# johanngerberding/voxelnet-pytorch

Hardware: AMD Instinct MI355X
Metric: point-clouds/sec fwd+bwd, KITTI car voxel grid, batch=2 (higher is better)
Workload: dtype bf16; 1 GPU; KITTI car config (voxel 0.2x0.2x0.4 m, grid 10x400x352, T=35), batch=2 per GPU, fwd+bwd train step (BASELINE configs[1]); global_batch=2, points_per_frame=19861, parallelism=dp1, launch_mode=eager+native-executor+one-call-step

## Files before the change

### voxelnet-pytorch_amd/csrc/conv.hip

```cpp
#include "common.h"

namespace {

constexpr int GG_MAX_TAPS = 32;
constexpr int GG_MAX_CLASSES = 16;
constexpr uint32_t GG_OOB = 0xFFFFF000u;
constexpr uint32_t GG_MAX_WINDOW = 0xFFFFE000u;

struct GGClass {
    int32_t tap_begin, ntaps;
    int32_t nD, nH, nW;
    int32_t qD, qH, qW;
    int32_t ooffD, ooffH, ooffW;
    int32_t offD[4], offH[4], offW[4];
};
struct GGTap {
    int32_t id, ih, iw, widx;
};
struct GGParams {
    const char *src;
    const char *w;
    const float *bias;
    char *out;
    float *stats;
// ... 10 lines not shown
    uint32_t w_bytes;
    int64_t src_batch_extent;
    const int64_t *row_list;
    const int32_t *row_count;
    int32_t row_cap;
    int32_t out_linear;
    int32_t ldivD, ldivH, ldivW;
    int32_t slotcD[4], slotcH[4], slotcW[4];
    GGClass cls[GG_MAX_CLASSES];
    GGTap taps[GG_MAX_TAPS];
};

typedef __attribute__((address_space(3))) void lds_void_t;
#ifdef VN_P2D_TRACE
__device__ long long g_p2d_trace[64 * 8];
#define P2D_STAMP(s, k) do { if (tr_on) g_p2d_trace[((s) & 63) * 8 + (k)] = __builtin_amdgcn_s_memtime(); } while (0)
#else
#define P2D_STAMP(s, k) do {} while (0)
#endif
#ifndef GG_PIN_SCHEDULE
#define GG_PIN_SCHEDULE 1
#endif
#if GG_PIN_SCHEDULE
#define GG_PIN() __builtin_amdgcn_sched_barrier(0)
#else
#define GG_PIN()
#endif

__device__ __forceinline__ void lds_dma16(__amdgpu_buffer_rsrc_t rsrc, char *lds_wave_base, uint32_t voffset,
                                          uint32_t soffset) {
    __builtin_amdgcn_raw_ptr_buffer_load_lds(rsrc, (lds_void_t *)lds_wave_base, 16, voffset, soffset, 0, 0);
}

__device__ __forceinline__ void x3_weights(bool presplit, const char *g0, const char *g1, bf16x8_t &hi, bf16x8_t &lo) {
    if (presplit) {
        hi = *reinterpret_cast<const bf16x8_t *>(g0);
        lo = *reinterpret_cast<const bf16x8_t *>(g1);
    } else {
        vn_split8(*reinterpret_cast<const f32x4_t *>(g0), *reinterpret_cast<const f32x4_t *>(g1), hi, lo);
    }
}

template <int NT>
__device__ __forceinline__ void x3_split_patch(char *patch, int rows) {
    for (int item = threadIdx.x; item < rows * 4; item += NT) {
        const int q = item >> 2, f = item & 3, sw = (q >> 1) & 7;
        char *g0 = patch + q * 128 + (((2 * f) ^ sw) << 4), *g1 = patch + q * 128 + (((2 * f + 1) ^ sw) << 4);
        bf16x8_t hi, lo;
        vn_split8(*reinterpret_cast<const f32x4_t *>(g0), *reinterpret_cast<const f32x4_t *>(g1), hi, lo);
        *reinterpret_cast<bf16x8_t *>(g0) = hi;
        *reinterpret_cast<bf16x8_t *>(g1) = lo;
    }
}

template <int WM, int WN, int SM, bool BNBWD = false>
__device__ __forceinline__ void gg_store(const GGParams &p, f32x4_t (&acc)[SM][4], char *smem, const int32_t *otab, int64_t tile,
                                         int n0, int wm, int wn, int lane) {
    constexpr int BN = 64 * WN;
    const int fr = lane & 15, fq = lane >> 4;
    const int64_t tile_m = tile;
    const int ncol = n0 + wn * 64 + fr * 4;
    const bool col_ok = ncol < p.N;
    float bias4[4] = {0.f, 0.f, 0.f, 0.f};
    if (p.bias && col_ok) {
        const float4 bv = *reinterpret_cast<const float4 *>(p.bias + ncol);
        bias4[0] = bv.x; bias4[1] = bv.y; bias4[2] = bv.z; bias4[3] = bv.w;
    }
    float s1[4] = {0.f, 0.f, 0.f, 0.f}, s2[4] = {0.f, 0.f, 0.f, 0.f};
    float bmean[4] = {0.f, 0.f, 0.f, 0.f}, binv[4] = {0.f, 0.f, 0.f, 0.f}, bS[4] = {0.f, 0.f, 0.f, 0.f}, bbe[4] = {0.f, 0.f, 0.f, 0.f};
    if constexpr (BNBWD) {
        if (col_ok) {
#pragma unroll
            for (int j = 0; j < 4; ++j) {
                bmean[j] = p.bn_stats[ncol + j]; binv[j] = p.bn_stats[p.N + ncol + j];
                bS[j] = p.bn_stats[2 * p.N + ncol + j]; bbe[j] = p.bn_stats[3 * p.N + ncol + j];
            }
        }
    }
#pragma unroll
    for (int i = 0; i < SM; ++i) {
        const int4 offs = *reinterpret_cast<const int4 *>(otab + wm * (16 * SM) + i * 16 + fq * 4);
        const int32_t o4[4] = {offs.x, offs.y, offs.z, offs.w};
#pragma unroll
        for (int e = 0; e < 4; ++e) {
            if (o4[e] < 0 || !col_ok) continue;
            float v[4];
            if constexpr (BNBWD) {
                float yv[4];
                if (p.bn_y_f32) {
                    const float4 t = *reinterpret_cast<const float4 *>(reinterpret_cast<const float *>(p.bn_y) + (int64_t)o4[e] + ncol);
                    yv[0] = t.x; yv[1] = t.y; yv[2] = t.z; yv[3] = t.w;
                } else {
                    const bf16x4_t t = *reinterpret_cast<const bf16x4_t *>(reinterpret_cast<const bf16_t *>(p.bn_y) + (int64_t)o4[e] + ncol);
#pragma unroll
                    for (int j = 0; j < 4; ++j) yv[j] = (float)t[j];
                }
#pragma unroll
                for (int j = 0; j < 4; ++j) {
                    const float a = acc[i][j][e];
                    v[j] = a;
                    const float st = p.out_f32 ? a : (float)(bf16_t)a;
                    const float d0 = yv[j] - bmean[j];
                    const float z = fmaf(bS[j], d0, bbe[j]);
                    const float dz = z > 0.f ? st : 0.f;
                    s1[j] += dz;
                    s2[j] += dz * (d0 * binv[j]);
                }
            } else {
#pragma unroll
            for (int j = 0; j < 4; ++j) {
                const float a = acc[i][j][e];
                s1[j] += a;
                s2[j] += a * a;
                v[j] = a + bias4[j];
            }
            }
            if (p.out_f32) {
                float4 *dst = reinterpret_cast<float4 *>(reinterpret_cast<float *>(p.out) + (int64_t)o4[e] + ncol);
                if (p.accumulate) {
                    const float4 old = *dst;
                    v[0] += old.x; v[1] += old.y; v[2] += old.z; v[3] += old.w;
                }
                *dst = make_float4(v[0], v[1], v[2], v[3]);
            } else {
                bf16x4_t *dst = reinterpret_cast<bf16x4_t *>(reinterpret_cast<bf16_t *>(p.out) + (int64_t)o4[e] + ncol);
                if (p.accumulate) {
                    const bf16x4_t old = *dst;
#pragma unroll
                    for (int j = 0; j < 4; ++j) v[j] += (float)old[j];
                }
                bf16x4_t o;
#pragma unroll
                for (int j = 0; j < 4; ++j) o[j] = (bf16_t)v[j];
                *dst = o;
            }
        }
    }
    if (p.stats) {
        __syncthreads();
        float *red = reinterpret_cast<float *>(smem);
#pragma unroll
        for (int j = 0; j < 4; ++j) {
            s1[j] += __shfl_xor(s1[j], 16, 64);
            s1[j] += __shfl_xor(s1[j], 32, 64);
            s2[j] += __shfl_xor(s2[j], 16, 64);
            s2[j] += __shfl_xor(s2[j], 32, 64);
        }
        if (fq == 0) {
#pragma unroll
            for (int j = 0; j < 4; ++j) {
                red[(wm * 2 + 0) * BN + wn * 64 + fr * 4 + j] = s1[j];
                red[(wm * 2 + 1) * BN + wn * 64 + fr * 4 + j] = s2[j];
            }
        }
        __syncthreads();
        for (int i = threadIdx.x; i < 2 * BN; i += 64 * WM * WN) {
            const int which = i / BN, c = i - which * BN;
            float v = 0.f;
#pragma unroll
            for (int w = 0; w < WM; ++w) v += red[(w * 2 + which) * BN + c];
            if (n0 + c < p.N) p.stats[((int64_t)tile_m * 2 + which) * p.N + n0 + c] = v;
        }
    }
}

template <int WM, int WN, int SM, int NS, bool F32>
__global__ void __launch_bounds__(256, 2) k_gather_gemm(const GGParams p) {
    VN_PRIO_MAIN();
    static_assert(WM * WN == 4 && NS >= 2 && SM >= 1 && SM <= 8, "4 waves");
    constexpr int ESZ = F32 ? 4 : 2;
    constexpr int BM = 16 * SM * WM, BN = 64 * WN;
    static_assert(BM % 32 == 0, "a DMA instruction of the 4 waves covers 32 rows");
    constexpr int RA = BM / 32, RB = BN / 32;
    constexpr int A_BYTES = BM * 128, B_BYTES = BN * 128, STAGE = A_BYTES + B_BYTES;
    constexpr int AHEAD = (NS - 2) * (RA + RB);
    static_assert(AHEAD <= 63, "vmcnt is 6 bits");
    extern __shared__ __attribute__((aligned(16))) char smem[];

    const int lane = threadIdx.x & 63;
    const int wave = __builtin_amdgcn_readfirstlane(threadIdx.x >> 6);
    const int wm = wave / WN, wn = wave % WN;

    const GGClass &cl = p.cls[blockIdx.y];
    const int ntn = (p.N + BN - 1) / BN;
    int bid = blockIdx.x;
    {
        const int nwg = gridDim.x, q = nwg >> 3, r = nwg & 7, x = bid & 7;
        bid = (x < r ? x * (q + 1) : r * (q + 1) + (x - r) * q) + (bid >> 3);
    }
    const int tile_m = bid / ntn, tile_n = bid - tile_m * ntn;
    const int qD = cl.qD, qH = cl.qH, qW = cl.qW;
    const bool list = p.row_list != nullptr;
    const int64_t Mq = list ? (p.row_count ? (int64_t)p.row_count[0] : (int64_t)p.row_cap) : (int64_t)p.B * qD * qH * qW;
    const int64_t m0 = (int64_t)tile_m * BM;
    const int n0 = tile_n * BN;
    if (m0 >= Mq) {
// ... 227 lines not shown
        nbuf = nbuf + 1 == NS ? 0 : nbuf + 1;
    }

    __syncthreads();
    int32_t *otab = reinterpret_cast<int32_t *>(smem);
    for (int r = threadIdx.x; r < BM; r += 256) {
        const int64_t m = m0 + r;
        int32_t off = -1;
        if (m < Mq && list) {
            if (p.out_linear) {
                off = (int32_t)(m * p.oW);
            } else {
                const int64_t *rc = p.row_list + m * 4;
                off = (int32_t)(rc[0] * p.oB + rc[1] * p.oD + rc[2] * p.oH + rc[3] * p.oW);
            }
        } else if (m < Mq) {
            int t = (int)(m % rows_per_b);
            const int b = (int)(m / rows_per_b);
            const int qw = t % qW;
            t /= qW;
            const int qh = t % qH;
            const int qd = t / qH;
            const int od = qd * p.omulD + cl.ooffD, oh = qh * p.omulH + cl.ooffH, ow = qw * p.omulW + cl.ooffW;
            if (od < p.Do && oh < p.Ho && ow < p.Wo)
                off = (int32_t)((int64_t)b * p.oB + (int64_t)od * p.oD + (int64_t)oh * p.oH + (int64_t)ow * p.oW);
        }
        otab[r] = off;
    }
    __syncthreads();

    gg_store<WM, WN, SM>(p, acc, smem, otab, (int64_t)blockIdx.y * (gridDim.x / ntn) + tile_m, n0, wm, wn, lane);
}

template <int WM, int WN, int SM, int TW, bool F32>
__global__ void __launch_bounds__(256, 2) k_conv_patch(const GGParams p) {
    VN_PRIO_MAIN();
    constexpr int ESZ = F32 ? 4 : 2;
    constexpr int BM = 16 * SM * WM, BN = 64 * WN, TH = BM / TW;
    static_assert(WM * WN == 4 && BM % TW == 0, "4 waves; whole patch lines");
    constexpr int PW = TW + 2, PH = TH + 2, PROWS = PH * PW;
    constexpr int PPIECES = (PROWS + 7) / 8;
    constexpr int PA = (PPIECES + 3) / 4;
    constexpr int PATCH_BYTES = PA * 4 * 1024;
    constexpr int RB = BN / 32;
    constexpr int B_BYTES = BN * 128;
    extern __shared__ __attribute__((aligned(16))) char smem[];
    char *patch = smem;
    char *bst = smem + PATCH_BYTES;

    const int lane = threadIdx.x & 63;
    const int wave = __builtin_amdgcn_readfirstlane(threadIdx.x >> 6);
    const int wm = wave / WN, wn = wave % WN;
    const GGClass &cl = p.cls[blockIdx.y];
    const int ntn = (p.N + BN - 1) / BN;
    int bid = blockIdx.x;
    {
        const int nwg = gridDim.x, q = nwg >> 3, r = nwg & 7, x = bid & 7;
        bid = (x < r ? x * (q + 1) : r * (q + 1) + (x - r) * q) + (bid >> 3);
    }
    const int tile = bid / ntn, tile_n = bid - tile * ntn;
    const int n0 = tile_n * BN;
    const int tiles_x = (cl.qW + TW - 1) / TW, tiles_y = (cl.qH + TH - 1) / TH;
    int t = tile;
    const int tx = t % tiles_x; t /= tiles_x;
    const int ty = t % tiles_y; t /= tiles_y;
    const int qd = t % cl.qD;
// ... 7 lines not shown
    for (int i = 0; i < PA; ++i) {
        const int q = (i * 4 + wave) * 8 + (lane >> 3);
        const int qy = q / PW, qx = q - qy * PW;
        const int sy = y0 - 1 + qy, sx = x0 - 1 + qx;
        a_row[i] = (q < PROWS && (unsigned)sy < (unsigned)p.Hs && (unsigned)sx < (unsigned)p.Ws)
                       ? (uint32_t)(((int64_t)sy * p.sH + (int64_t)sx * p.sW) * ESZ)
                       : GG_OOB;
    }
    uint32_t b_row[RB];
#pragma unroll
    for (int i = 0; i < RB; ++i) {
        const int rho = (i * 4 + wave) * 8 + (lane >> 3);
        const int rl = rho & 63;
        const int n = n0 + (rho & ~63) + (rl & 15) * 4 + (rl >> 4);
        b_row[i] = n < p.N ? (uint32_t)((int64_t)n * p.Cs * ESZ) : GG_OOB;
    }
    const char *src_base = p.src + (int64_t)b * p.sB * ESZ;
    int64_t src_bytes = p.src_batch_extent * ESZ;
    if (src_bytes > (int64_t)GG_MAX_WINDOW) src_bytes = GG_MAX_WINDOW;
    const __amdgpu_buffer_rsrc_t rs_a = vn_uniform_rsrc(src_base, (uint32_t)src_bytes);
    const __amdgpu_buffer_rsrc_t rs_b = vn_uniform_rsrc(p.w, p.w_bytes);
    constexpr int BKE = 128 / ESZ, EPC = 16 / ESZ;
    const int nk = (p.Cs + BKE - 1) / BKE;
    const int k_lane0 = a_chunk * EPC;

    const int fr = lane & 15, fq = lane >> 4;
    int q0[SM];
#pragma unroll
    for (int i = 0; i < SM; ++i) {
        const int r = wm * (16 * SM) + i * 16 + fr;
        const int py = r / TW, px = r - py * TW;
        q0[i] = (py + 1) * PW + (px + 1);
    }
    const int bfrag0 = fr * 128 + (((0 + fq) ^ (fr >> 1)) << 4);
    const int bfrag1 = fr * 128 + (((4 + fq) ^ (fr >> 1)) << 4);
    const int x3_b0 = fr * 128 + (((2 * fq) ^ (fr >> 1)) << 4);
    const int x3_b1 = fr * 128 + (((2 * fq + 1) ^ (fr >> 1)) << 4);

    f32x4_t acc[SM][4];
#pragma unroll
    for (int i = 0; i < SM; ++i)
#pragma unroll
        for (int j = 0; j < 4; ++j) acc[i][j] = f32x4_t{0.f, 0.f, 0.f, 0.f};

    const uint32_t tap_bytes = (uint32_t)p.N * (uint32_t)p.Cs * (uint32_t)ESZ;
    auto wbase_of = [&](int id) { return p.taps[cl.tap_begin + id * 9].widx; };
    auto stage_b = [&](int wbase, int tap, int kc, int buf) {
        const int k_lane = kc * BKE + k_lane0;
        const bool k_ok = k_lane < p.Cs;
        const uint32_t b_koff = (uint32_t)k_lane * (uint32_t)ESZ;
        const uint32_t b_soff = __builtin_amdgcn_readfirstlane((uint32_t)(wbase + tap) * tap_bytes);
        char *lb = bst + buf * B_BYTES + wave * 1024;
#pragma unroll
        for (int i = 0; i < RB; ++i)
            lds_dma16(rs_b, lb + i * 4096, (k_ok && b_row[i] != GG_OOB) ? b_row[i] + b_koff : GG_OOB, b_soff);
    };
    auto stage_patch = [&](int sd, int kc) {
        const int k_lane = kc * BKE + k_lane0;
        const bool k_ok = k_lane < p.Cs;
        const int k_src = k_lane;
        const uint32_t off = (uint32_t)(((int64_t)sd * p.sD + k_src) * ESZ);
#pragma unroll
        for (int i = 0; i < PA; ++i)
            lds_dma16(rs_a, patch + (i * 4 + wave) * 1024, (k_ok && a_row[i] != GG_OOB) ? a_row[i] + off : GG_OOB, 0);
    };

    int bbuf = 0;
    bool first = true;
    for (int id = 0; id < cl.nD; ++id) {
        const int sd = qd * p.mulD + cl.offD[id];
        if ((unsigned)sd >= (unsigned)p.Ds) continue;
        const int wbase = wbase_of(id);
        for (int kc = 0; kc < nk; ++kc) {
            __syncthreads();
            stage_patch(sd, kc);
            if (first) { stage_b(wbase, 0, kc, bbuf); first = false; }
            for (int tap = 0; tap < 9; ++tap) {
                const int ih = tap / 3, iw = tap - ih * 3;
                asm volatile("s_waitcnt vmcnt(0) lgkmcnt(0)" ::: "memory");
                __builtin_amdgcn_s_barrier();
                asm volatile("" ::: "memory");
                if (tap < 8) {
                    stage_b(wbase, tap + 1, kc, bbuf ^ 1);
                } else {
                    int nid = id, nkc = kc + 1;
                    if (nkc == nk) {
                        nkc = 0;
                        for (nid = id + 1; nid < cl.nD; ++nid)
                            if ((unsigned)(qd * p.mulD + cl.offD[nid]) < (unsigned)p.Ds) break;
                    }
                    if (nid < cl.nD) stage_b(nid == id ? wbase : wbase_of(nid), 0, nkc, bbuf ^ 1);
                }
                const int shift = cl.offH[ih] * PW + cl.offW[iw];
                const char *lb = bst + bbuf * B_BYTES + wn * (64 * 128);
                bool x3_done = false;
                if constexpr (F32) {
                    if (p.x3) {
                        if (tap == 0 && p.x3 != 3) {
                            x3_split_patch<256>(patch, PA * 32);
                            asm volatile("s_waitcnt lgkmcnt(0)" ::: "memory");
                            __builtin_amdgcn_s_barrier();
                            asm volatile("" ::: "memory");
                        }
                        bf16x8_t bh[4], bl[4];
#pragma unroll
                        for (int j = 0; j < 4; ++j) x3_weights(p.x3 >= 2, lb + j * 2048 + x3_b0, lb + j * 2048 + x3_b1, bh[j], bl[j]);
#pragma unroll
                        for (int i = 0; i < SM; ++i) {
                            const int q = q0[i] + shift;
                            const bf16x8_t ah = *reinterpret_cast<const bf16x8_t *>(patch + q * 128 + (((2 * fq) ^ ((q >> 1) & 7)) << 4));
                            const bf16x8_t al = *reinterpret_cast<const bf16x8_t *>(patch + q * 128 + (((2 * fq + 1) ^ ((q >> 1) & 7)) << 4));
#pragma unroll
                            for (int j = 0; j < 4; ++j) acc[i][j] = vn_mfma_x3(ah, al, bh[j], bl[j], acc[i][j]);
                        }
                        x3_done = true;
                    }
                }
                if (!x3_done) {
#pragma unroll
                for (int ks = 0; ks < 2; ++ks) {
                    const int fo = ks ? bfrag1 : bfrag0;
                    if constexpr (F32) {
                        f32x4_t bq[4];
#pragma unroll
                        for (int j = 0; j < 4; ++j) bq[j] = *reinterpret_cast<const f32x4_t *>(lb + j * 2048 + fo);
#pragma unroll
                        for (int i = 0; i < SM; ++i) {
                            const int q = q0[i] + shift;
                            const f32x4_t a = *reinterpret_cast<const f32x4_t *>(patch + q * 128 + (((ks * 4 + fq) ^ ((q >> 1) & 7)) << 4));
#pragma unroll
                            for (int t4 = 0; t4 < 4; ++t4)
#pragma unroll
                                for (int j = 0; j < 4; ++j)
                                    acc[i][j] = __builtin_amdgcn_mfma_f32_16x16x4f32(a[t4], bq[j][t4], acc[i][j], 0, 0, 0);
                        }
                    } else {
                        bf16x8_t bq[4];
#pragma unroll
                        for (int j = 0; j < 4; ++j) bq[j] = *reinterpret_cast<const bf16x8_t *>(lb + j * 2048 + fo);
#pragma unroll
                        for (int i = 0; i < SM; ++i) {
                            const int q = q0[i] + shift;
                            const bf16x8_t a = *reinterpret_cast<const bf16x8_t *>(patch + q * 128 + (((ks * 4 + fq) ^ ((q >> 1) & 7)) << 4));
#pragma unroll
                            for (int j = 0; j < 4; ++j)
                                acc[i][j] = __builtin_amdgcn_mfma_f32_16x16x32_bf16(a, bq[j], acc[i][j], 0, 0, 0);
                        }
                    }
                }
                }
                bbuf ^= 1;
            }
        }
    }

    __syncthreads();
    int32_t *otab = reinterpret_cast<int32_t *>(smem);
    for (int r = threadIdx.x; r < BM; r += 256) {
        const int py = r / TW, px = r - py * TW;
        const int qh = y0 + py, qw = x0 + px;
        int32_t off = -1;
        if (qh < cl.qH && qw < cl.qW) {
            const int od = qd * p.omulD + cl.ooffD, oh = qh * p.omulH + cl.ooffH, ow = qw * p.omulW + cl.ooffW;
            if (od < p.Do && oh < p.Ho && ow < p.Wo)
                off = (int32_t)((int64_t)b * p.oB + (int64_t)od * p.oD + (int64_t)oh * p.oH + (int64_t)ow * p.oW);
        }
        otab[r] = off;
    }
    __syncthreads();
    gg_store<WM, WN, SM>(p, acc, smem, otab, tile, n0, wm, wn, lane);
}

template <int WM, int WN, int SM, int TW, int NSB, bool F32>
__global__ void __launch_bounds__(64 * WM * WN, WM * WN == 4 ? 2 : 1) k_conv_patch2d(const GGParams p) {
    VN_PRIO_MAIN();
    constexpr int ESZ = F32 ? 4 : 2;
    constexpr int NW = WM * WN, NT = 64 * NW;
    constexpr int BM = 16 * SM * WM, BN = 64 * WN, TH = BM / TW;
    static_assert((NW == 4 || NW == 8) && BM % TW == 0 && (BN / 8) % NW == 0, "4 or 8 waves; whole patch lines");
    constexpr int PW = TW + 2, PH = TH + 2, PROWS = PH * PW;
    constexpr int PPIECES = (PROWS + 7) / 8;
    constexpr int PA = (PPIECES + NW - 1) / NW;
    constexpr int PATCH_BYTES = PA * NW * 1024;
    constexpr int RB = BN / (8 * NW);
    constexpr int B_BYTES = BN * 128;
    extern __shared__ __attribute__((aligned(16))) char smem[];
    char *bst = smem + 2 * PATCH_BYTES;
    static_assert(NSB >= 3 && (NSB - 2) * RB <= 63, "vmcnt is 6 bits");

    const int lane = threadIdx.x & 63;
    const int wave = __builtin_amdgcn_readfirstlane(threadIdx.x >> 6);
    const int wm = wave / WN, wn = wave % WN;
    const GGClass &cl = p.cls[blockIdx.y];
    const int ntn = (p.N + BN - 1) / BN;
    int bid = blockIdx.x;
    {
        const int nwg = gridDim.x, q = nwg >> 3, r = nwg & 7, x = bid & 7;
        bid = (x < r ? x * (q + 1) : r * (q + 1) + (x - r) * q) + (bid >> 3);
    }
    const int tile = bid / ntn, tile_n = bid - tile * ntn;
    const int n0 = tile_n * BN;
    const int tiles_x = (cl.qW + TW - 1) / TW, tiles_y = (cl.qH + TH - 1) / TH;
    int t = tile;
// ... 255 lines not shown
    if (Cr <= 64) return GG_CFG[0];
    const int64_t b1 = blocks(GG_CFG[1]), b4 = blocks(GG_CFG[4]);
    if (b1 < 100) return GG_CFG[2];
    const int64_t t1 = vn_ceil_div(b1, 512) * 128, t4 = vn_ceil_div(b4, 512) * 160;
    return t4 < t1 ? GG_CFG[4] : GG_CFG[1];
}

struct PatchCfg {
    int id, BM, BN, TW;
};
int patch_enabled() {
    static const int v = vn_knob("VN_PATCH", 1);
    return v;
}
PatchCfg patch_config(const vnConv *g) {
    PatchCfg none{-1, 0, 0, 0};
    if (!patch_enabled()) return none;
    if (g->kH != 3 || g->kW != 3 || g->mulH != 1 || g->mulW != 1 || g->divH != 1 || g->divW != 1) return none;
    if (!((g->tmulH == 1 && g->padH == 1) || (g->tmulH == -1 && g->padH == -1))) return none;
    if (!((g->tmulW == 1 && g->padW == 1) || (g->tmulW == -1 && g->padW == -1))) return none;
    if (g->src_wrap != 0 || (g->Cr & 63)) return none;
    if (g->Hs != g->Hr || g->Ws != g->Wr) return none;
    if (g->Hr < 128 || g->Wr < 128) {
        if (patch_enabled() == 3 || g->Cr == 64) return none;
        return PatchCfg{2, 64, 128, 16};
    }
    if (g->Cr == 64) return PatchCfg{3, 192, 64, 32};
    return PatchCfg{0, 160, 128, 16};
}
int64_t patch_tiles(const PatchCfg &c, int B, int qD, int qH, int qW) {
    const int TH = c.BM / c.TW;
    return (int64_t)B * qD * vn_ceil_div(qH, TH) * vn_ceil_div(qW, c.TW);
}
template <int WM, int WN, int SM, int TW, bool F32>
int launch_patch(const GGParams &p, dim3 grid, hipStream_t st) {
    constexpr int BM = 16 * SM * WM, TH = BM / TW, PROWS = (TH + 2) * (TW + 2);
    constexpr size_t lds = (size_t)((PROWS + 7) / 8 + 3) / 4 * 4096 + 2 * (size_t)(64 * WN) * 128;
    static const hipError_t attr = hipFuncSetAttribute(reinterpret_cast<const void *>(&k_conv_patch<WM, WN, SM, TW, F32>),
                                                       hipFuncAttributeMaxDynamicSharedMemorySize, (int)lds);
    if (attr != hipSuccess) return (int)attr;
    k_conv_patch<WM, WN, SM, TW, F32><<<grid, 256, lds, st>>>(p);
    return 0;
}
template <int WM, int WN, int SM, int TW, int NSB, bool F32>
int launch_patch2d(const GGParams &p, dim3 grid, hipStream_t st) {
    constexpr int BM = 16 * SM * WM, TH = BM / TW, PROWS = (TH + 2) * (TW + 2), NW = WM * WN;
    constexpr size_t lds = 2 * ((size_t)((PROWS + 7) / 8 + NW - 1) / NW * NW * 1024) + NSB * (size_t)(64 * WN) * 128;
    static const hipError_t attr = hipFuncSetAttribute(reinterpret_cast<const void *>(&k_conv_patch2d<WM, WN, SM, TW, NSB, F32>),
                                                       hipFuncAttributeMaxDynamicSharedMemorySize, (int)lds);
    if (attr != hipSuccess) return (int)attr;
    k_conv_patch2d<WM, WN, SM, TW, NSB, F32><<<grid, 64 * NW, lds, st>>>(p);
    return 0;
}
int patch2d_stages() {
    static const int v = vn_knob("VN_PATCH2D", 3);
    return v;
}
int launch_patch_cfg(const PatchCfg &c, bool f32, const GGParams &p, dim3 grid, hipStream_t st) {
    if (c.id == 2 && p.Ds == 1 && p.nclasses == 1 && p.cls[0].nD == 1 && patch2d_stages() >= 3) {
        const GGParams &q = p;
        if (patch2d_stages() == 3 && !f32) return launch_patch2d<4, 2, 1, 16, 3, false>(q, grid, st);
        if (patch2d_stages() == 3 && f32 && q.x3) return launch_patch2d<4, 2, 1, 16, 3, true>(q, grid, st);
        if (patch2d_stages() == 3)
            return f32 ? launch_patch2d<2, 2, 2, 16, 3, true>(q, grid, st) : launch_patch2d<2, 2, 2, 16, 3, false>(q, grid, st);
        return f32 ? launch_patch2d<2, 2, 2, 16, 4, true>(q, grid, st) : launch_patch2d<2, 2, 2, 16, 4, false>(q, grid, st);
    }
    if (c.id == 3) return f32 ? launch_patch<4, 1, 3, 32, true>(p, grid, st) : launch_patch<4, 1, 3, 32, false>(p, grid, st);
    if (c.id == 2) return f32 ? launch_patch<2, 2, 2, 16, true>(p, grid, st) : launch_patch<2, 2, 2, 16, false>(p, grid, st);
    return f32 ? launch_patch<2, 2, 5, 16, true>(p, grid, st) : launch_patch<2, 2, 5, 16, false>(p, grid, st);
}

int launch_cfg(const GGConfig &c, bool f32, const GGParams &p, dim3 grid, hipStream_t st) {
    switch (c.id) {
    case 0: return f32 ? launch_gg<4, 1, 4, 2, true>(p, grid, st) : launch_gg<4, 1, 4, 2, false>(p, grid, st);
    case 1: return f32 ? launch_gg<2, 2, 4, 2, true>(p, grid, st) : launch_gg<2, 2, 4, 2, false>(p, grid, st);
    case 2: return f32 ? launch_gg<2, 2, 2, 4, true>(p, grid, st) : launch_gg<2, 2, 2, 4, false>(p, grid, st);
    case 3: return f32 ? launch_gg<4, 1, 1, 6, true>(p, grid, st) : launch_gg<4, 1, 1, 6, false>(p, grid, st);
    default: return f32 ? launch_gg<2, 2, 5, 2, true>(p, grid, st) : launch_gg<2, 2, 5, 2, false>(p, grid, st);
    }
}

struct AxisSlots {
    int n, cls[4], off[4], tap[4];
};
bool axis_slots(int k, int tmul, int pad, int div, AxisSlots *o) {
    o->n = 0;
    for (int r = 0; r < div; ++r)
        for (int t = 0; t < k; ++t) {
            const int num = r + t * tmul - pad;
            if (posmod(num, div) != 0) continue;
            if (o->n >= 4) return false;
            o->cls[o->n] = div == 1 ? -1 : r;
            o->off[o->n] = floordiv(num, div);
            o->tap[o->n] = t;
            ++o->n;
        }
    return o->n > 0;
}

}
// ... 69 lines not shown
        c.offH[j] = j < sh.n ? sh.off[j] : (1 << 29);
        c.offW[j] = j < sw.n ? sw.off[j] : (1 << 29);
        p.slotcD[j] = j < sd.n ? sd.cls[j] : -2;
        p.slotcH[j] = j < sh.n ? sh.cls[j] : -2;
        p.slotcW[j] = j < sw.n ? sw.cls[j] : -2;
    }
    int ntap = 0;
    for (int i = 0; i < sd.n; ++i)
        for (int j = 0; j < sh.n; ++j)
            for (int k = 0; k < sw.n; ++k)
                p.taps[ntap++] = GGTap{i, j, k, (sd.tap[i] * g->kH + sh.tap[j]) * g->kW + sw.tap[k]};
    c.ntaps = ntap;
    p.nclasses = 1;
    const GGConfig cfg = g->Cr > 64 ? GG_CFG[1] : GG_CFG[0];
    const int64_t tiles_m = vn_ceil_div(row_cap, cfg.BM), tiles_n = vn_ceil_div(g->Cr, cfg.BN);
    const dim3 grid((unsigned)(tiles_m * tiles_n), 1);
    hipStream_t st = vn_stream(stream);
    const int rc = launch_cfg(cfg, f32, p, grid, st);
    if (rc) return rc;
    VN_LAUNCH_STATUS();
    return VN_OK;
}

extern "C" int64_t vn_conv_stats_slab_rows(const vnConv *g) {
    if (!g || g->divD < 1 || g->divH < 1 || g->divW < 1) return 0;
    if (g->divD * g->divH * g->divW > 1) {
        const int64_t qd = vn_ceil_div(g->Dr, g->divD), qh = vn_ceil_div(g->Hr, g->divH), qw = vn_ceil_div(g->Wr, g->divW);
        const int nd = g->divD < g->Dr ? g->divD : g->Dr, nh = g->divH < g->Hr ? g->divH : g->Hr, nw = g->divW < g->Wr ? g->divW : g->Wr;
        const int64_t rows = (int64_t)g->B * qd * qh * qw;
        const int ncls = nd * nh * nw;
        return (int64_t)ncls * vn_ceil_div(rows, gg_config(rows, g->Cr, ncls).BM);
    }
    const PatchCfg pc = patch_config(g);
    if (pc.id >= 0) return patch_tiles(pc, g->B, g->Dr, g->Hr, g->Wr);
    const int64_t rows = (int64_t)g->B * g->Dr * g->Hr * g->Wr;
    return vn_ceil_div(rows, gg_config(rows, g->Cr, 1).BM);
}

extern "C" int32_t vn_conv_plan_id(const vnConv *g) {
    if (!g || g->divD < 1 || g->divH < 1 || g->divW < 1 || g->B <= 0) return -1;
    const PatchCfg pc = patch_config(g);
    if (pc.id == 2 && g->Ds == 1 && g->Dr == 1 && g->kD == 1 && g->divD == 1 && patch2d_stages() >= 3)
        return 120 + patch2d_stages();
    if (pc.id >= 0) return 100 + pc.id;
    const int64_t qd = vn_ceil_div(g->Dr, g->divD), qh = vn_ceil_div(g->Hr, g->divH), qw = vn_ceil_div(g->Wr, g->divW);
    const int nd = g->divD < g->Dr ? g->divD : g->Dr, nh = g->divH < g->Hr ? g->divH : g->Hr, nw = g->divW < g->Wr ? g->divW : g->Wr;
    return gg_config((int64_t)g->B * qd * qh * qw, g->Cr, nd * nh * nw).id;
}

static int gather_gemm_impl(const void *src, const void *w_packed, const float *bias, void *out, vnDtype out_dtype,
                            const vnConv *g, int32_t accumulate, float *stats_slab, vnStream stream, const void *bn_y,
                            vnDtype bn_y_dtype, const float *bn_stats);

extern "C" int vn_conv_gather_gemm(const void *src, const void *w_packed, const float *bias, void *out,
                                   vnDtype out_dtype, const vnConv *g, int32_t accumulate, float *stats_slab,
                                   vnStream stream) {
    return gather_gemm_impl(src, w_packed, bias, out, out_dtype, g, accumulate, stats_slab, stream, nullptr, VN_BF16, nullptr);
}

extern "C" int vn_conv_dgrad_bn_bwd(const void *src, const void *w_packed, void *out, vnDtype out_dtype, const vnConv *g,
                                    const void *bn_y, vnDtype bn_y_dtype, const float *bn_stats, float *slab,
                                    vnStream stream) {
    VN_CHECK_ARG(bn_y && bn_stats && slab && g);
    if (vn_conv_plan_id(g) != 123) return VN_EUNSUPPORTED;
    return gather_gemm_impl(src, w_packed, nullptr, out, out_dtype, g, 0, slab, stream, bn_y, bn_y_dtype, bn_stats);
}

// ... 67 lines not shown
            for (int cw = 0; cw < ncw; ++cw) {
                const AxisClass &D = ad[cd], &H = ah[ch], &W = aw[cw];
                GGClass &c = p.cls[ncls];
                c.tap_begin = ntap;
                c.nD = D.n; c.nH = H.n; c.nW = W.n;
                c.qD = D.q; c.qH = H.q; c.qW = W.q;
                c.ooffD = D.r; c.ooffH = H.r; c.ooffW = W.r;
                for (int j = 0; j < 4; ++j) {
                    c.offD[j] = j < D.n ? D.off[j] : (1 << 29);
                    c.offH[j] = j < H.n ? H.off[j] : (1 << 29);
                    c.offW[j] = j < W.n ? W.off[j] : (1 << 29);
                }
                for (int i = 0; i < D.n; ++i)
                    for (int j = 0; j < H.n; ++j)
                        for (int k = 0; k < W.n; ++k) {
                            if (ntap >= GG_MAX_TAPS) return VN_EUNSUPPORTED;
                            p.taps[ntap++] = GGTap{i, j, k, (D.tap[i] * g->kH + H.tap[j]) * g->kW + W.tap[k]};
                        }
                c.ntaps = ntap - c.tap_begin;
                const int64_t rows = (int64_t)g->B * D.q * H.q * W.q;
                if (rows > max_rows) max_rows = rows;
                ++ncls;
            }
    p.nclasses = ncls;

    const PatchCfg pc = patch_config(g);
    if (pc.id >= 0) {
        int64_t tiles = 0;
        for (int c = 0; c < ncls; ++c) {
            const int64_t t = patch_tiles(pc, g->B, p.cls[c].qD, p.cls[c].qH, p.cls[c].qW);
            if (t > tiles) tiles = t;
        }
        if (p.src_batch_extent * esz > (int64_t)GG_MAX_WINDOW - 4096) return VN_EUNSUPPORTED;
        const int64_t nblk = tiles * vn_ceil_div(g->Cr, pc.BN);
        if (nblk > 0x7fffffffll) return VN_EUNSUPPORTED;
        const dim3 pgrid((unsigned)nblk, (unsigned)ncls);
        const int prc = launch_patch_cfg(pc, f32, p, pgrid, vn_stream(stream));
        if (prc) return prc;
        VN_LAUNCH_STATUS();
        return VN_OK;
    }
    const GGConfig cfg = gg_config(max_rows, g->Cr, ncls);
    const int BM = cfg.BM, BN = cfg.BN;
    {
        int64_t min_rows_b = (int64_t)p.cls[0].qD * p.cls[0].qH * p.cls[0].qW;
        for (int c = 1; c < ncls; ++c) {
            const int64_t r = (int64_t)p.cls[c].qD * p.cls[c].qH * p.cls[c].qW;
            if (r < min_rows_b) min_rows_b = r;
        }
        if (min_rows_b <= 0) min_rows_b = 1;
        int64_t span_b = BM / min_rows_b + 2;
        if (span_b > g->B) span_b = g->B;
        const int64_t need = ((span_b - 1) * g->src_sB + p.src_batch_extent) * esz;
        if (need > (int64_t)GG_MAX_WINDOW - 4096) return VN_EUNSUPPORTED;
    }
    const int64_t tiles_m = vn_ceil_div(max_rows, BM);
    const int64_t tiles_n = vn_ceil_div(g->Cr, BN);
    if (tiles_m * tiles_n > 0x7fffffffll) return VN_EUNSUPPORTED;
    const dim3 grid((unsigned)(tiles_m * tiles_n), (unsigned)ncls);
    hipStream_t st = vn_stream(stream);
    const int rc = launch_cfg(cfg, f32, p, grid, st);
    if (rc) return rc;
    VN_LAUNCH_STATUS();
    return VN_OK;
}

#ifdef VN_P2D_TRACE
extern "C" int vn_debug_p2d_trace(long long *out ) {
    return (int)hipMemcpyFromSymbol(out, HIP_SYMBOL(g_p2d_trace), sizeof(long long) * 64 * 8);
}
#endif
```

Measured before the change: 569.2 point-clouds/s.

## Make bf16 patch conv persistent over tiles with cross-tile weight/patch prefetch

```diff
diff --git a/voxelnet-pytorch_amd/csrc/conv.hip b/voxelnet-pytorch_amd/csrc/conv.hip
--- a/voxelnet-pytorch_amd/csrc/conv.hip
+++ b/voxelnet-pytorch_amd/csrc/conv.hip
@@ -66,6 +66,12 @@
     __builtin_amdgcn_raw_ptr_buffer_load_lds(rsrc, (lds_void_t *)lds_wave_base, 16, voffset, soffset, 0, 0);
 }
 
+__device__ __forceinline__ void lds_barrier() {
+    asm volatile("s_waitcnt lgkmcnt(0)" ::: "memory");
+    __builtin_amdgcn_s_barrier();
+    asm volatile("" ::: "memory");
+}
+
 __device__ __forceinline__ void x3_weights(bool presplit, const char *g0, const char *g1, bf16x8_t &hi, bf16x8_t &lo) {
     if (presplit) {
         hi = *reinterpret_cast<const bf16x8_t *>(g0);
@@ -87,20 +93,22 @@
     }
 }
 
-template <int WM, int WN, int SM, bool BNBWD = false>
-__device__ __forceinline__ void gg_store(const GGParams &p, f32x4_t (&acc)[SM][4], char *smem, const int32_t *otab, int64_t tile,
-                                         int n0, int wm, int wn, int lane) {
-    constexpr int BN = 64 * WN;
+__device__ __forceinline__ void gg_load_bias(const GGParams &p, int n0, int wn, int lane, float (&bias4)[4]) {
+    const int ncol = n0 + wn * 64 + (lane & 15) * 4;
+    bias4[0] = bias4[1] = bias4[2] = bias4[3] = 0.f;
+    if (p.bias && ncol < p.N) {
+        const float4 bv = *reinterpret_cast<const float4 *>(p.bias + ncol);
+        bias4[0] = bv.x; bias4[1] = bv.y; bias4[2] = bv.z; bias4[3] = bv.w;
+    }
+    asm volatile("" : "+v"(bias4[0]), "+v"(bias4[1]), "+v"(bias4[2]), "+v"(bias4[3]));
+}
+
+template <int WM, int WN, int SM, bool BNBWD = false, class OT>
+__device__ __forceinline__ void gg_store_rows(const GGParams &p, f32x4_t (&acc)[SM][4], const OT &row_offs, int n0, int wm, int wn,
+                                              int lane, const float (&bias4)[4], float (&s1)[4], float (&s2)[4]) {
     const int fr = lane & 15, fq = lane >> 4;
-    const int64_t tile_m = tile;
     const int ncol = n0 + wn * 64 + fr * 4;
     const bool col_ok = ncol < p.N;
-    float bias4[4] = {0.f, 0.f, 0.f, 0.f};
-    if (p.bias && col_ok) {
-        const float4 bv = *reinterpret_cast<const float4 *>(p.bias + ncol);
-        bias4[0] = bv.x; bias4[1] = bv.y; bias4[2] = bv.z; bias4[3] = bv.w;
-    }
-    float s1[4] = {0.f, 0.f, 0.f, 0.f}, s2[4] = {0.f, 0.f, 0.f, 0.f};
     float bmean[4] = {0.f, 0.f, 0.f, 0.f}, binv[4] = {0.f, 0.f, 0.f, 0.f}, bS[4] = {0.f, 0.f, 0.f, 0.f}, bbe[4] = {0.f, 0.f, 0.f, 0.f};
     if constexpr (BNBWD) {
         if (col_ok) {
@@ -113,7 +121,7 @@
     }
 #pragma unroll
     for (int i = 0; i < SM; ++i) {
-        const int4 offs = *reinterpret_cast<const int4 *>(otab + wm * (16 * SM) + i * 16 + fq * 4);
+        const int4 offs = row_offs(wm * (16 * SM) + i * 16 + fq * 4);
         const int32_t o4[4] = {offs.x, offs.y, offs.z, offs.w};
 #pragma unroll
         for (int e = 0; e < 4; ++e) {
@@ -170,6 +178,14 @@
             }
         }
     }
+}
+
+template <int WM, int WN>
+__device__ __forceinline__ void gg_store_stats(const GGParams &p, char *smem, int64_t tile, int n0, int wm, int wn, int lane,
+                                               float (&s1)[4], float (&s2)[4]) {
+    constexpr int BN = 64 * WN;
+    const int fr = lane & 15, fq = lane >> 4;
+    const int64_t tile_m = tile;
     if (p.stats) {
         __syncthreads();
         float *red = reinterpret_cast<float *>(smem);
@@ -196,6 +212,16 @@
             if (n0 + c < p.N) p.stats[((int64_t)tile_m * 2 + which) * p.N + n0 + c] = v;
         }
     }
+}
+
+template <int WM, int WN, int SM, bool BNBWD = false>
+__device__ __forceinline__ void gg_store(const GGParams &p, f32x4_t (&acc)[SM][4], char *smem, const int32_t *otab, int64_t tile,
+                                         int n0, int wm, int wn, int lane) {
+    float s1[4] = {0.f, 0.f, 0.f, 0.f}, s2[4] = {0.f, 0.f, 0.f, 0.f}, bias4[4];
+    gg_load_bias(p, n0, wn, lane, bias4);
+    gg_store_rows<WM, WN, SM, BNBWD>(p, acc, [&](int r) { return *reinterpret_cast<const int4 *>(otab + r); }, n0, wm, wn, lane,
+                                     bias4, s1, s2);
+    gg_store_stats<WM, WN>(p, smem, tile, n0, wm, wn, lane, s1, s2);
 }
 
 template <int WM, int WN, int SM, int NS, bool F32>
@@ -489,6 +515,69 @@
     gg_store<WM, WN, SM>(p, acc, smem, otab, (int64_t)blockIdx.y * (gridDim.x / ntn) + tile_m, n0, wm, wn, lane);
 }
 
+template <int SM, int PW, int PA, bool F32>
+__device__ __forceinline__ void patch_tap_mfma(const GGParams &p, const GGClass &cl, char *patch, const char *lb, int tap,
+                                               const int (&q0)[SM], int fq, const int (&fo4)[4], f32x4_t (&acc)[SM][4]) {
+    const int ih = tap / 3, iw = tap - ih * 3;
+    const int shift = cl.offH[ih] * PW + cl.offW[iw];
+    bool x3_done = false;
+    if constexpr (F32) {
+        if (p.x3) {
+            if (tap == 0 && p.x3 != 3) {
+                x3_split_patch<256>(patch, PA * 32);
+                asm volatile("s_waitcnt lgkmcnt(0)" ::: "memory");
+                __builtin_amdgcn_s_barrier();
+                asm volatile("" ::: "memory");
+            }
+            bf16x8_t bh[4], bl[4];
+#pragma unroll
+            for (int j = 0; j < 4; ++j) x3_weights(p.x3 >= 2, lb + j * 2048 + fo4[2], lb + j * 2048 + fo4[3], bh[j], bl[j]);
+#pragma unroll
+            for (int i = 0; i < SM; ++i) {
+                const int q = q0[i] + shift;
+                const bf16x8_t ah = *reinterpret_cast<const bf16x8_t *>(patch + q * 128 + (((2 * fq) ^ ((q >> 1) & 7)) << 4));
+                const bf16x8_t al = *reinterpret_cast<const bf16x8_t *>(patch + q * 128 + (((2 * fq + 1) ^ ((q >> 1) & 7)) << 4));
+#pragma unroll
+                for (int j = 0; j < 4; ++j) acc[i][j] = vn_mfma_x3(ah, al, bh[j], bl[j], acc[i][j]);
+            }
+            x3_done = true;
+        }
+    }
+    if (!x3_done) {
+#pragma unroll
+    for (int ks = 0; ks < 2; ++ks) {
+        const int fo = fo4[ks];
+        if constexpr (F32) {
+            f32x4_t bq[4];
+#pragma unroll
+            for (int j = 0; j < 4; ++j) bq[j] = *reinterpret_cast<const f32x4_t *>(lb + j * 2048 + fo);
+#pragma unroll
+            for (int i = 0; i < SM; ++i) {
+                const int q = q0[i] + shift;
+                const f32x4_t a = *reinterpret_cast<const f32x4_t *>(patch + q * 128 + (((ks * 4 + fq) ^ ((q >> 1) & 7)) << 4));
+#pragma unroll
+                for (int t4 = 0; t4 < 4; ++t4)
+#pragma unroll
+                    for (int j = 0; j < 4; ++j)
+                        acc[i][j] = __builtin_amdgcn_mfma_f32_16x16x4f32(a[t4], bq[j][t4], acc[i][j], 0, 0, 0);
+            }
+        } else {
+            bf16x8_t bq[4];
+#pragma unroll
+            for (int j = 0; j < 4; ++j) bq[j] = *reinterpret_cast<const bf16x8_t *>(lb + j * 2048 + fo);
+#pragma unroll
+            for (int i = 0; i < SM; ++i) {
+                const int q = q0[i] + shift;
+                const bf16x8_t a = *reinterpret_cast<const bf16x8_t *>(patch + q * 128 + (((ks * 4 + fq) ^ ((q >> 1) & 7)) << 4));
+#pragma unroll
+                for (int j = 0; j < 4; ++j)
+                    acc[i][j] = __builtin_amdgcn_mfma_f32_16x16x32_bf16(a, bq[j], acc[i][j], 0, 0, 0);
+            }
+        }
+    }
+    }
+}
+
 template <int WM, int WN, int SM, int TW, bool F32>
 __global__ void __launch_bounds__(256, 2) k_conv_patch(const GGParams p) {
     VN_PRIO_MAIN();
@@ -562,10 +651,8 @@
         const int py = r / TW, px = r - py * TW;
         q0[i] = (py + 1) * PW + (px + 1);
     }
-    const int bfrag0 = fr * 128 + (((0 + fq) ^ (fr >> 1)) << 4);
-    const int bfrag1 = fr * 128 + (((4 + fq) ^ (fr >> 1)) << 4);
-    const int x3_b0 = fr * 128 + (((2 * fq) ^ (fr >> 1)) << 4);
-    const int x3_b1 = fr * 128 + (((2 * fq + 1) ^ (fr >> 1)) << 4);
+    const int fo4[4] = {fr * 128 + (((0 + fq) ^ (fr >> 1)) << 4), fr * 128 + (((4 + fq) ^ (fr >> 1)) << 4),
+                        fr * 128 + (((2 * fq) ^ (fr >> 1)) << 4), fr * 128 + (((2 * fq + 1) ^ (fr >> 1)) << 4)};
 
     f32x4_t acc[SM][4];
 #pragma unroll
@@ -606,7 +693,6 @@
             stage_patch(sd, kc);
             if (first) { stage_b(wbase, 0, kc, bbuf); first = false; }
             for (int tap = 0; tap < 9; ++tap) {
-                const int ih = tap / 3, iw = tap - ih * 3;
                 asm volatile("s_waitcnt vmcnt(0) lgkmcnt(0)" ::: "memory");
                 __builtin_amdgcn_s_barrier();
                 asm volatile("" ::: "memory");
@@ -621,64 +707,7 @@
                     }
                     if (nid < cl.nD) stage_b(nid == id ? wbase : wbase_of(nid), 0, nkc, bbuf ^ 1);
                 }
-                const int shift = cl.offH[ih] * PW + cl.offW[iw];
-                const char *lb = bst + bbuf * B_BYTES + wn * (64 * 128);
-                bool x3_done = false;
-                if constexpr (F32) {
-                    if (p.x3) {
-                        if (tap == 0 && p.x3 != 3) {
-                            x3_split_patch<256>(patch, PA * 32);
-                            asm volatile("s_waitcnt lgkmcnt(0)" ::: "memory");
-                            __builtin_amdgcn_s_barrier();
-                            asm volatile("" ::: "memory");
-                        }
-                        bf16x8_t bh[4], bl[4];
-#pragma unroll
-                        for (int j = 0; j < 4; ++j) x3_weights(p.x3 >= 2, lb + j * 2048 + x3_b0, lb + j * 2048 + x3_b1, bh[j], bl[j]);
-#pragma unroll
-                        for (int i = 0; i < SM; ++i) {
-                            const int q = q0[i] + shift;
-                            const bf16x8_t ah = *reinterpret_cast<const bf16x8_t *>(patch + q * 128 + (((2 * fq) ^ ((q >> 1) & 7)) << 4));
-                            const bf16x8_t al = *reinterpret_cast<const bf16x8_t *>(patch + q * 128 + (((2 * fq + 1) ^ ((q >> 1) & 7)) << 4));
-#pragma unroll
-                            for (int j = 0; j < 4; ++j) acc[i][j] = vn_mfma_x3(ah, al, bh[j], bl[j], acc[i][j]);
-                        }
-                        x3_done = true;
-                    }
-                }
-                if (!x3_done) {
-#pragma unroll
-                for (int ks = 0; ks < 2; ++ks) {
-                    const int fo = ks ? bfrag1 : bfrag0;
-                    if constexpr (F32) {
-                        f32x4_t bq[4];
-#pragma unroll
-                        for (int j = 0; j < 4; ++j) bq[j] = *reinterpret_cast<const f32x4_t *>(lb + j * 2048 + fo);
-#pragma unroll
-                        for (int i = 0; i < SM; ++i) {
-                            const int q = q0[i] + shift;
-                            const f32x4_t a = *reinterpret_cast<const f32x4_t *>(patch + q * 128 + (((ks * 4 + fq) ^ ((q >> 1) & 7)) << 4));
-#pragma unroll
-                            for (int t4 = 0; t4 < 4; ++t4)
-#pragma unroll
-                                for (int j = 0; j < 4; ++j)
-                                    acc[i][j] = __builtin_amdgcn_mfma_f32_16x16x4f32(a[t4], bq[j][t4], acc[i][j], 0, 0, 0);
-                        }
-                    } else {
-                        bf16x8_t bq[4];
-#pragma unroll
-                        for (int j = 0; j < 4; ++j) bq[j] = *reinterpret_cast<const bf16x8_t *>(lb + j * 2048 + fo);
-#pragma unroll
-                        for (int i = 0; i < SM; ++i) {
-                            const int q = q0[i] + shift;
-                            const bf16x8_t a = *reinterpret_cast<const bf16x8_t *>(patch + q * 128 + (((ks * 4 + fq) ^ ((q >> 1) & 7)) << 4));
-#pragma unroll
-                            for (int j = 0; j < 4; ++j)
-                                acc[i][j] = __builtin_amdgcn_mfma_f32_16x16x32_bf16(a, bq[j], acc[i][j], 0, 0, 0);
-                        }
-                    }
-                }
-                }
+                patch_tap_mfma<SM, PW, PA, F32>(p, cl, patch, bst + bbuf * B_BYTES + wn * (64 * 128), tap, q0, fq, fo4, acc);
                 bbuf ^= 1;
             }
         }
@@ -699,6 +728,196 @@
     }
     __syncthreads();
     gg_store<WM, WN, SM>(p, acc, smem, otab, tile, n0, wm, wn, lane);
+}
+
+template <int WM, int WN, int SM, int TW, bool F32>
+__global__ void __launch_bounds__(256, 3) k_conv_patch_tiles(const GGParams p) {
+    VN_PRIO_MAIN();
+    constexpr int ESZ = F32 ? 4 : 2;
+    constexpr int BM = 16 * SM * WM, BN = 64 * WN, TH = BM / TW;
+    static_assert(WM * WN == 4 && BM % TW == 0, "4 waves; whole patch lines");
+    constexpr int PW = TW + 2, PH = TH + 2, PROWS = PH * PW;
+    constexpr int PPIECES = (PROWS + 7) / 8;
+    constexpr int PA = (PPIECES + 3) / 4;
+    constexpr int PATCH_BYTES = PA * 4 * 1024;
+    constexpr int RB = BN / 32;
+    constexpr int B_BYTES = BN * 128;
+    extern __shared__ __attribute__((aligned(16))) char smem[];
+    char *patch = smem;
+    char *bst = smem + PATCH_BYTES;
+
+    const int lane = threadIdx.x & 63;
+    const int wave = __builtin_amdgcn_readfirstlane(threadIdx.x >> 6);
+    const int wm = wave / WN, wn = wave % WN;
+    const GGClass &cl = p.cls[blockIdx.y];
+    const int ntn = (p.N + BN - 1) / BN;
+    int bid = blockIdx.x;
+    {
+        const int nwg = gridDim.x, q = nwg >> 3, r = nwg & 7, x = bid & 7;
+        bid = (x < r ? x * (q + 1) : r * (q + 1) + (x - r) * q) + (bid >> 3);
+    }
+    const int nwg_t = gridDim.x / ntn;
+    const int wg = bid / ntn, tile_n = bid - wg * ntn;
+    const int n0 = tile_n * BN;
+    const int tiles_x = (cl.qW + TW - 1) / TW, tiles_y = (cl.qH + TH - 1) / TH;
+    const int ntiles = p.B * cl.qD * tiles_y * tiles_x;
+    const int64_t slab_row = (int64_t)blockIdx.y * nwg_t + wg;
+
+    const int a_chunk = (lane & 7) ^ ((wave * 4 + (lane >> 4)) & 7);
+    uint32_t b_row[RB];
+#pragma unroll
+    for (int i = 0; i < RB; ++i) {
+        const int rho = (i * 4 + wave) * 8 + (lane >> 3);
+        const int rl = rho & 63;
+        const int n = n0 + (rho & ~63) + (rl & 15) * 4 + (rl >> 4);
+        b_row[i] = n < p.N ? (uint32_t)((int64_t)n * p.Cs * ESZ) : GG_OOB;
+    }
+    int64_t src_bytes = p.src_batch_extent * ESZ;
+    if (src_bytes > (int64_t)GG_MAX_WINDOW) src_bytes = GG_MAX_WINDOW;
+    const __amdgpu_buffer_rsrc_t rs_b = vn_uniform_rsrc(p.w, p.w_bytes);
+    constexpr int BKE = 128 / ESZ, EPC = 16 / ESZ;
+    const int nk = (p.Cs + BKE - 1) / BKE;
+    const int k_lane0 = a_chunk * EPC;
+
+    const int fr = lane & 15, fq = lane >> 4;
+    int q0[SM];
+#pragma unroll
+    for (int i = 0; i < SM; ++i) {
+        const int r = wm * (16 * SM) + i * 16 + fr;
+        const int py = r / TW, px = r - py * TW;
+        q0[i] = (py + 1) * PW + (px + 1);
+    }
+    const int fo4[4] = {fr * 128 + (((0 + fq) ^ (fr >> 1)) << 4), fr * 128 + (((4 + fq) ^ (fr >> 1)) << 4),
+                        fr * 128 + (((2 * fq) ^ (fr >> 1)) << 4), fr * 128 + (((2 * fq + 1) ^ (fr >> 1)) << 4)};
+
+    const uint32_t tap_bytes = (uint32_t)p.N * (uint32_t)p.Cs * (uint32_t)ESZ;
+    auto wbase_of = [&](int id) { return p.taps[cl.tap_begin + id * 9].widx; };
+    auto stage_b = [&](int wbase, int tap, int kc, int buf) {
+        const int k_lane = kc * BKE + k_lane0;
+        const bool k_ok = k_lane < p.Cs;
+        const uint32_t b_koff = (uint32_t)k_lane * (uint32_t)ESZ;
+        const uint32_t b_soff = __builtin_amdgcn_readfirstlane((uint32_t)(wbase + tap) * tap_bytes);
+        char *lb = bst + buf * B_BYTES + wave * 1024;
+#pragma unroll
+        for (int i = 0; i < RB; ++i)
+            lds_dma16(rs_b, lb + i * 4096, (k_ok && b_row[i] != GG_OOB) ? b_row[i] + b_koff : GG_OOB, b_soff);
+    };
+
+    struct Tile { int b, qd, y0, x0; };
+    auto tile_at = [&](int tile) {
+        int t = tile;
+        const int tx = t % tiles_x; t /= tiles_x;
+        const int ty = t % tiles_y; t /= tiles_y;
+        const int qd = t % cl.qD;
+        return Tile{t / cl.qD, qd, ty * TH, tx * TW};
+    };
+    auto first_plane = [&](int qd, int from) {
+        int id = from;
+        for (; id < cl.nD; ++id)
+            if ((unsigned)(qd * p.mulD + cl.offD[id]) < (unsigned)p.Ds) break;
+        return id;
+    };
+    uint32_t a_row[PA];
+    __amdgpu_buffer_rsrc_t rs_a;
+    auto set_tile = [&](const Tile &tl) {
+#pragma unroll
+        for (int i = 0; i < PA; ++i) {
+            const int q = (i * 4 + wave) * 8 + (lane >> 3);
+            const int qy = q / PW, qx = q - qy * PW;
+            const int sy = tl.y0 - 1 + qy, sx = tl.x0 - 1 + qx;
+            a_row[i] = (q < PROWS && (unsigned)sy < (unsigned)p.Hs && (unsigned)sx < (unsigned)p.Ws)
+                           ? (uint32_t)(((int64_t)sy * p.sH + (int64_t)sx * p.sW) * ESZ)
+                           : GG_OOB;
+        }
+        rs_a = vn_uniform_rsrc(p.src + (int64_t)tl.b * p.sB * ESZ, (uint32_t)src_bytes);
+    };
+    auto stage_patch = [&](int sd, int kc) {
+        const int k_lane = kc * BKE + k_lane0;
+        const bool k_ok = k_lane < p.Cs;
+        const int k_src = k_lane;
+        const uint32_t off = (uint32_t)(((int64_t)sd * p.sD + k_src) * ESZ);
+#pragma unroll
+        for (int i = 0; i < PA; ++i)
+            lds_dma16(rs_a, patch + (i * 4 + wave) * 1024, (k_ok && a_row[i] != GG_OOB) ? a_row[i] + off : GG_OOB, 0);
+    };
+
+    float s1[4] = {0.f, 0.f, 0.f, 0.f}, s2[4] = {0.f, 0.f, 0.f, 0.f};
+    float bias4[4];
+    gg_load_bias(p, n0, wn, lane, bias4);
+    int bbuf = 0;
+    bool staged = false;
+    for (int tile = wg; tile < ntiles; tile += nwg_t) {
+        const Tile tl = tile_at(tile);
+        const int qd = tl.qd;
+        const bool has_next = tile + nwg_t < ntiles;
+        const Tile nx = tile_at(has_next ? tile + nwg_t : tile);
+        const int nx_id = has_next ? first_plane(nx.qd, 0) : cl.nD;
+        if (!staged) set_tile(tl);
+
+        f32x4_t acc[SM][4];
+#pragma unroll
+        for (int i = 0; i < SM; ++i)
+#pragma unroll
+            for (int j = 0; j < 4; ++j) acc[i][j] = f32x4_t{0.f, 0.f, 0.f, 0.f};
+
+        bool first = !staged, ran = false;
+        for (int id = 0; id < cl.nD; ++id) {
+            const int sd = qd * p.mulD + cl.offD[id];
+            if ((unsigned)sd >= (unsigned)p.Ds) continue;
+            const int wbase = wbase_of(id);
+            for (int kc = 0; kc < nk; ++kc) {
+                if (!staged) {
+                    __syncthreads();
+                    stage_patch(sd, kc);
+                    if (first) { stage_b(wbase, 0, kc, bbuf); first = false; }
+                }
+                staged = false;
+                ran = true;
+                for (int tap = 0; tap < 9; ++tap) {
+                    asm volatile("s_waitcnt vmcnt(0) lgkmcnt(0)" ::: "memory");
+                    __builtin_amdgcn_s_barrier();
+                    asm volatile("" ::: "memory");
+                    if (tap < 8) {
+                        stage_b(wbase, tap + 1, kc, bbuf ^ 1);
+                    } else {
+                        int nid = id, nkc = kc + 1;
+                        if (nkc == nk) {
+                            nkc = 0;
+                            nid = first_plane(qd, id + 1);
+                        }
+                        if (nid < cl.nD) stage_b(nid == id ? wbase : wbase_of(nid), 0, nkc, bbuf ^ 1);
+                        else if (nx_id < cl.nD) stage_b(wbase_of(nx_id), 0, 0, bbuf ^ 1);
+                    }
+                    patch_tap_mfma<SM, PW, PA, F32>(p, cl, patch, bst + bbuf * B_BYTES + wn * (64 * 128), tap, q0, fq, fo4, acc);
+                    bbuf ^= 1;
+                }
+            }
+        }
+
+        lds_barrier();
+        if (nx_id < cl.nD) {
+            set_tile(nx);
+            stage_patch(nx.qd * p.mulD + cl.offD[nx_id], 0);
+            if (!ran) stage_b(wbase_of(nx_id), 0, 0, bbuf);
+            staged = true;
+        }
+        const int od = qd * p.omulD + cl.ooffD;
+        const int32_t obase = (int32_t)((int64_t)tl.b * p.oB + (int64_t)od * p.oD);
+        auto row_offs = [&](int r0) {
+            int32_t o[4];
+#pragma unroll
+            for (int e = 0; e < 4; ++e) {
+                const int r = r0 + e, py = r / TW, px = r - py * TW;
+                const int qh = tl.y0 + py, qw = tl.x0 + px;
+                const int oh = qh * p.omulH + cl.ooffH, ow = qw * p.omulW + cl.ooffW;
+                const bool ok = qh < cl.qH && qw < cl.qW && od < p.Do && oh < p.Ho && ow < p.Wo;
+                o[e] = ok ? obase + (int32_t)((int64_t)oh * p.oH + (int64_t)ow * p.oW) : -1;
+            }
+            return make_int4(o[0], o[1], o[2], o[3]);
+        };
+        gg_store_rows<WM, WN, SM>(p, acc, row_offs, n0, wm, wn, lane, bias4, s1, s2);
+    }
+    gg_store_stats<WM, WN>(p, smem, slab_row, n0, wm, wn, lane, s1, s2);
 }
 
 template <int WM, int WN, int SM, int TW, int NSB, bool F32>
@@ -1020,6 +1239,15 @@
     const int TH = c.BM / c.TW;
     return (int64_t)B * qD * vn_ceil_div(qH, TH) * vn_ceil_div(qW, c.TW);
 }
+constexpr int PATCH_SLOTS = 256 * 3 * 2;
+int g_patch_slots_debug = 0;
+bool patch_persistent(const PatchCfg &c, bool f32) { return c.id == 3 && !f32; }
+int64_t patch_workgroups(const PatchCfg &c, bool f32, int64_t tiles) {
+    if (!patch_persistent(c, f32)) return tiles;
+    const int64_t slots = g_patch_slots_debug > 0 ? g_patch_slots_debug : PATCH_SLOTS;
+    const int64_t per = vn_ceil_div(tiles, slots);
+    return per > 0 ? vn_ceil_div(tiles, per) : 0;
+}
 template <int WM, int WN, int SM, int TW, bool F32>
 int launch_patch(const GGParams &p, dim3 grid, hipStream_t st) {
     constexpr int BM = 16 * SM * WM, TH = BM / TW, PROWS = (TH + 2) * (TW + 2);
@@ -1030,6 +1258,16 @@
     k_conv_patch<WM, WN, SM, TW, F32><<<grid, 256, lds, st>>>(p);
     return 0;
 }
+template <int WM, int WN, int SM, int TW, bool F32>
+int launch_patch_tiles(const GGParams &p, dim3 grid, hipStream_t st) {
+    constexpr int BM = 16 * SM * WM, TH = BM / TW, PROWS = (TH + 2) * (TW + 2);
+    constexpr size_t lds = (size_t)((PROWS + 7) / 8 + 3) / 4 * 4096 + 2 * (size_t)(64 * WN) * 128;
+    static const hipError_t attr = hipFuncSetAttribute(reinterpret_cast<const void *>(&k_conv_patch_tiles<WM, WN, SM, TW, F32>),
+                                                       hipFuncAttributeMaxDynamicSharedMemorySize, (int)lds);
+    if (attr != hipSuccess) return (int)attr;
+    k_conv_patch_tiles<WM, WN, SM, TW, F32><<<grid, 256, lds, st>>>(p);
+    return 0;
+}
 template <int WM, int WN, int SM, int TW, int NSB, bool F32>
 int launch_patch2d(const GGParams &p, dim3 grid, hipStream_t st) {
     constexpr int BM = 16 * SM * WM, TH = BM / TW, PROWS = (TH + 2) * (TW + 2), NW = WM * WN;
@@ -1053,7 +1291,7 @@
             return f32 ? launch_patch2d<2, 2, 2, 16, 3, true>(q, grid, st) : launch_patch2d<2, 2, 2, 16, 3, false>(q, grid, st);
         return f32 ? launch_patch2d<2, 2, 2, 16, 4, true>(q, grid, st) : launch_patch2d<2, 2, 2, 16, 4, false>(q, grid, st);
     }
-    if (c.id == 3) return f32 ? launch_patch<4, 1, 3, 32, true>(p, grid, st) : launch_patch<4, 1, 3, 32, false>(p, grid, st);
+    if (c.id == 3) return f32 ? launch_patch<4, 1, 3, 32, true>(p, grid, st) : launch_patch_tiles<4, 1, 3, 32, false>(p, grid, st);
     if (c.id == 2) return f32 ? launch_patch<2, 2, 2, 16, true>(p, grid, st) : launch_patch<2, 2, 2, 16, false>(p, grid, st);
     return f32 ? launch_patch<2, 2, 5, 16, true>(p, grid, st) : launch_patch<2, 2, 5, 16, false>(p, grid, st);
 }
@@ -1189,7 +1427,7 @@
         return (int64_t)ncls * vn_ceil_div(rows, gg_config(rows, g->Cr, ncls).BM);
     }
     const PatchCfg pc = patch_config(g);
-    if (pc.id >= 0) return patch_tiles(pc, g->B, g->Dr, g->Hr, g->Wr);
+    if (pc.id >= 0) return patch_workgroups(pc, g->dtype != VN_BF16, patch_tiles(pc, g->B, g->Dr, g->Hr, g->Wr));
     const int64_t rows = (int64_t)g->B * g->Dr * g->Hr * g->Wr;
     return vn_ceil_div(rows, gg_config(rows, g->Cr, 1).BM);
 }
@@ -1323,7 +1561,9 @@
             if (t > tiles) tiles = t;
         }
         if (p.src_batch_extent * esz > (int64_t)GG_MAX_WINDOW - 4096) return VN_EUNSUPPORTED;
-        const int64_t nblk = tiles * vn_ceil_div(g->Cr, pc.BN);
+        if (tiles > 0x7fffffffll) return VN_EUNSUPPORTED;
+        if (stats_slab && ncls > 1 && patch_persistent(pc, f32)) return VN_EUNSUPPORTED;
+        const int64_t nblk = patch_workgroups(pc, f32, tiles) * vn_ceil_div(g->Cr, pc.BN);
         if (nblk > 0x7fffffffll) return VN_EUNSUPPORTED;
         const dim3 pgrid((unsigned)nblk, (unsigned)ncls);
         const int prc = launch_patch_cfg(pc, f32, p, pgrid, vn_stream(stream));
@@ -1356,6 +1596,12 @@
     return VN_OK;
 }
 
+extern "C" int vn_debug_conv_patch_slots(int slots) {
+    const int old = g_patch_slots_debug;
+    g_patch_slots_debug = slots > 0 ? slots : 0;
+    return old;
+}
+
 #ifdef VN_P2D_TRACE
 extern "C" int vn_debug_p2d_trace(long long *out ) {
     return (int)hipMemcpyFromSymbol(out, HIP_SYMBOL(g_p2d_trace), sizeof(long long) * 64 * 8);
```

After: 565.7 point-clouds/s (median of 3 runs). Within noise of the previous version (-0.6%).
